# nintendops/DynamicFusion_Body

Hardware: AMD Instinct MI355X
Metric: Mvoxels/s TSDF fusion + GN-iters/s warp solve, 256³ grid, 1/2/4/8 GPU (higher is better)
Workload: dtype f64 geometry / f32 volume

## Files before the change

### dynamicfusion_body_amd/_lib.py

```python
import ctypes
import os
import re

_PKG = os.path.dirname(os.path.abspath(__file__))
LIB_PATH = os.environ.get("DFH_LIB_PATH") or os.path.join(_PKG, "libdfusion_hip.so")
HEADER_PATH = os.path.join(os.path.dirname(_PKG), "include", "dfusion_hip.h")

F32, F64 = 0, 1
ABI_VERSION = 8

_c_double_p = ctypes.POINTER(ctypes.c_double)
_c_int_p = ctypes.POINTER(ctypes.c_int)
_vp = ctypes.c_void_p
_int = ctypes.c_int
_dbl = ctypes.c_double


class Problem(ctypes.Structure):
    _fields_ = [("sample_pos", _vp), ("sample_nrm", _vp), ("nbr", _vp), ("weights", _vp), ("corr", _vp), ("valid", _vp),
                ("n_samples", _int), ("knn", _int),
                ("node_dq", _vp), ("node_pos", _vp), ("node_w", _vp), ("node_nbr", _vp), ("n_nodes", _int),
                ("lw_dq", _dbl * 8), ("rw", _dbl), ("huber_delta", _dbl),
                ("row_ptr", _vp), ("col", _vp), ("n_blocks", _int), ("vals", _vp), ("rhs", _vp), ("cost_count", _vp),
                ("blk_upper", _vp), ("n_upper", _int),
# ... 70 lines not shown
    "dfh_integrate_depth": (_int, [_volume_p, ctypes.POINTER(DepthViews), _dbl, _dbl, _c_double_p, _vp, ctypes.c_size_t, _vp]),
    "dfh_integrate_depth_path": (_int, [_int, _slab_p, _int, _int, _int]),
    "dfh_integrate_depth_ocl": (_int, [_volume_p, _vp, _int, _int, ctypes.POINTER(ctypes.c_float), ctypes.POINTER(ctypes.c_float), ctypes.c_float, ctypes.c_float, _vp]),
    "dfh_fuse_volume_rigid": (_int, [_volume_p, ctypes.POINTER(Live), _c_double_p, _dbl, _dbl, _vp]),
    "dfh_dqb_workspace_bytes": (ctypes.c_size_t, [_slab_p]),
    "dfh_dqb_workspace_bytes_cached": (ctypes.c_size_t, [_slab_p, _int, _int, _int]),
    "dfh_fuse_volume_dqb": (_int, [_volume_p, ctypes.POINTER(Live), ctypes.POINTER(Nodes), _c_double_p, _dbl, _dbl, _vp, ctypes.c_size_t, _int, _vp]),
    "dfh_integrate_depth_dqb": (_int, [_volume_p, ctypes.POINTER(DepthViews), ctypes.POINTER(Nodes), _c_double_p, _dbl, _dbl, _int, _vp,
                                      ctypes.c_size_t, _int, _vp]),
    "dfh_residual_rigid": (_int, [_vp, _vp, _vp, _int, _c_double_p, _vp, _vp]),
    "dfh_gn_build_rigid": (_int, [_vp, _vp, _vp, _vp, _int, _c_double_p, _vp, _vp]),
    "dfh_residual_data": (_int, [_vp, _vp, _vp, _vp, _int, _int, _vp, _vp, _vp, _int, _c_double_p, _vp, _vp]),
    "dfh_residual_reg": (_int, [_vp, _int, _int, _vp, _vp, _vp, _dbl, _vp, _vp]),
    "dfh_warp_points": (_int, [_vp, _vp, _vp, _int, _int, _vp, _vp, _vp, _int, _c_double_p, _vp, _vp, _vp]),
    "dfh_closest_correspondences": (_int, [_vp, _vp, _int, _vp, _int, _int, _dbl, _vp, _vp, _vp, _vp]),
    "dfh_nearest_points": (_int, [_vp, _int, _vp, _int, _vp, _vp, _vp]),
    "dfh_graph_unsupported": (_int, [_vp, _int, _vp, _int, _vp, _vp, _int, _vp, _vp]),
    "dfh_dq_blend_points": (_int, [_vp, _int, _vp, _int, _vp, _vp, _vp, _int, _vp, _vp]),
    "dfh_radius_sample_workspace_bytes": (ctypes.c_size_t, [ctypes.c_long]),
    "dfh_radius_sample": (_int, [_vp, ctypes.c_long, _dbl, _vp, ctypes.c_long, ctypes.POINTER(ctypes.c_long), _c_int_p, _vp,
                                 ctypes.c_size_t, _vp]),
    "dfh_sample_knn": (_int, [_vp, _int, _vp, _vp, _int, _int, _vp, _vp, _vp]),
    "dfh_dqb_skip_layout": (_int, [_slab_p, _c_int_p, _int, _int, ctypes.POINTER(ctypes.c_size_t)]),
    "dfh_dqb_build_candidates": (_int, [_slab_p, _vp, _int, _int, _vp, ctypes.c_size_t, _vp]),
    "dfh_sample_knn_bricks": (_int, [_vp, _int, _vp, _vp, _int, _int, _slab_p, _vp, ctypes.c_size_t, _vp, _vp, _vp]),
    "dfh_permute_samples": (_int, [_vp, _int, _int, _vp, _vp, _vp, _vp, _vp, _vp, _vp, _vp, _vp]),
    "dfh_gn_partial_doubles": (ctypes.c_size_t, [_int]),
    "dfh_gn_views_bytes": (ctypes.c_size_t, [_int, _int, _int, _int]),
    "dfh_gn_pack_views": (_int, [_vp, _int, ctypes.POINTER(ctypes.c_void_p), _int, _int, _int, _c_double_p, _vp]),
    "dfh_gn_associate": (_int, [_problem_p, _frame_p, _vp]),
    "dfh_gn_associate_volume": (_int, [_problem_p, _term_p, _vp]),
    "dfh_gn_build": (_int, [_problem_p, _frame_p, _vp]),
    "dfh_gn_build_volume": (_int, [_problem_p, _term_p, _vp]),
    "dfh_gn_solve": (_int, [_problem_p, _frame_p, ctypes.POINTER(SolveParams), _vp]),
    "dfh_gn_solve_volume": (_int, [_problem_p, _term_p, ctypes.POINTER(SolveParams), _vp]),
    "dfh_gn_associate_gated": (_int, [_problem_p, _frame_p, _gate_p, _vp]),
    "dfh_gn_build_gated": (_int, [_problem_p, _frame_p, _gate_p, _vp]),
    "dfh_gn_solve_gated": (_int, [_problem_p, _frame_p, _gate_p, ctypes.POINTER(SolveParams), _vp]),
    "dfh_gn_global_sampled_gated": (_int, [_problem_p, _frame_p, _gate_p, _int, _dbl, _int, _vp, _vp, _vp, ctypes.c_size_t, _vp]),
    "dfh_gn_pack_upper": (_int, [_vp, _vp, _vp, _vp, _int, _int, _int, _vp, _vp]),
    "dfh_gn_unpack_upper": (_int, [_vp, _vp, _vp, _vp, _int, _int, _int, _vp, _vp]),
    "dfh_gn_sort_workspace_bytes": (ctypes.c_size_t, [_int]),
    "dfh_gn_sort_samples": (_int, [_vp, _vp, _vp, _vp, _int, _int, _int, _vp, _vp, _vp, _vp, _vp, _vp, _vp, ctypes.c_size_t, _vp]),
    "dfh_gn_tile_samples": (_int, []),
    "dfh_gn_plan_count": (_int, [_vp, _int, _int, _vp, _vp, _vp]),
    "dfh_gn_plan_workspace_bytes": (ctypes.c_size_t, [_int, _int]),
# ... 134 lines not shown
```

### dynamicfusion_body_amd/csrc/dfh_fuse_volume.hip

```cpp
#include "dfh_dqb_front.h"

#include <algorithm>
#include <cmath>
#include <cstdlib>
#include <mutex>
#include <unordered_map>

namespace dfh {

template <typename T, int N>
struct alignas(sizeof(T) * N) VPack {
    T v[N];
};

struct RigidParams {
    DQ lw;
    double tdist, wmax;
    int X, Y, Z;
    int LX, LY, LZ;
    int x0, nx;
    int zpacks, zp_shift;
};

__device__ __forceinline__ void pack_coords2(int zpacks, int zp_shift, int &y, int &zp) {
// ... 701 lines not shown
        if (DFH_K3_STUB & 16) in.idx = make_uint2((unsigned)(r & 255) | 0x10000u * ((r + 7) & 255), (unsigned)((r + 3) & 255) | 0x10000u * ((r + 11) & 255));
        else in.idx = *reinterpret_cast<const uint2 *>(knn_cache + off * 4);
        if (DFH_K3_STUB & 4) { in.w0 = 0.4 + 1e-9 * lane; in.w1 = 0.3; in.w2 = 0.2; in.wi = 30.0f; }
        else {
            in.w0 = w_cache[off]; in.w1 = w_cache[nvox + off]; in.w2 = w_cache[2 * nvox + off];
            in.wi = wi_cache[off];
        }
        in.t = tsdf[off]; in.w = tsdf_w[off];
    };
    auto coords = [&](int r, double &px, double &py, double &pz) {
        const int row = r / runs_per_row;
        const int xl = row / p.Y;
        px = (double)(p.x0 + xl); py = (double)(row - xl * p.Y); pz = (double)((r - row * runs_per_row) * 64 + lane);
    };
    auto nodes_of = [&](uint2 idx, int (&bi)[4]) {
        bi[0] = min((int)(idx.x & 0xffffu), p.N - 1); bi[1] = min((int)(idx.x >> 16), p.N - 1);
        bi[2] = min((int)(idx.y & 0xffffu), p.N - 1); bi[3] = min((int)(idx.y >> 16), p.N - 1);
    };
    if (LIST) {
        const int l = wave % kSkipLists, first = wave / kSkipLists, step = max(n_waves / kSkipLists, 1);
        if (wave >= step * kSkipLists) return;
        const unsigned *__restrict__ mine = list + (size_t)l * sub_cap;
        const int n_entries = (int)min(list_count[16 * l], sub_cap);
        const int n_items = 16 * ((n_entries + 3) >> 2);
        const unsigned last_brick = (unsigned)(p.nbx * p.nby * p.nbz - 1);
        const int g = lane >> 4;
        auto entry_of = [&](int it) { const int e = 4 * (it >> 4) + g; return e < n_entries ? min(mine[e], last_brick) : 0xffffffffu; };
        unsigned entry = first < n_items ? entry_of(first) : 0xffffffffu;
        for (int it = first; it < n_items; it += step) {
            const unsigned brick = entry;
            if (it + step < n_items) entry = entry_of(it + step);
            const int rr = it & 15;
            const bool have = brick != 0xffffffffu;
            const unsigned bq = have ? brick : 0u;
            const int bz = (int)(bq % (unsigned)p.nbz), bxy = (int)(bq / (unsigned)p.nbz);
            const int by = bxy % p.nby, bx = bxy / p.nby;
            const int xl = bx * kBX + (rr >> 2), y = by * kBY + (rr & 3);
            const bool valid = have && xl < p.nx && y < p.Y;
            const size_t off = ((size_t)xl * p.Y + y) * p.Z + (size_t)(bz * kBZ + (lane & 15));
            const double px = (double)(p.x0 + xl), py = (double)y, pz = (double)(bz * kBZ + (lane & 15));
            DqbRunInputs in;
            in.idx = make_uint2(0u, 0u); in.w0 = 1.0; in.w1 = in.w2 = 0.0; in.wi = 1.0f; in.t = in.w = 0.0f;
            if (valid) {
                in.idx = *reinterpret_cast<const uint2 *>(knn_cache + off * 4);
                in.w0 = w_cache[off]; in.w1 = w_cache[nvox + off]; in.w2 = w_cache[2 * nvox + off];
                in.wi = wi_cache[off];
                in.t = tsdf[off]; in.w = tsdf_w[off];
            }
            int bi[4];
            nodes_of(in.idx, bi);
            DqbNorm e;
            e.w0 = in.w0; e.w1 = in.w1; e.w2 = in.w2; e.wi = in.wi;
            DqbWarped wp = dqb_stage_warp(DqLds<STRIDE>{sdq}, bi, e, p, f, px, py, pz);
            if (!valid) { wp.ok = false; wp.redo = false; wp.fx = wp.fy = wp.fz = 0.0; }
            LiveT c[8];
            dqb_stage_gather(live, p, wp, c);
            dqb_stage_finish<LiveT, true>(tsdf, tsdf_w, live, node_pos, node_dq, node_w, bi, e.wi, p, wp, c, px, py, pz, off, in.t, in.w, redo_list);
        }
        return;
    }
    if (wave >= n_runs) return;
    for (int r = wave; r < n_runs; r += n_waves) {
        DqbRunInputs in;
// ... 23 lines not shown
        const size_t off = redo_list.offs[i];
        const int z = (int)(off % (size_t)p.Z);
        const int y = (int)((off / (size_t)p.Z) % (size_t)p.Y);
        const int xl = (int)(off / ((size_t)p.Z * p.Y));
        const uint2 v = *reinterpret_cast<const uint2 *>(knn_cache + off * 4);
        int bi[4];
        bi[0] = min((int)(v.x & 0xffffu), p.N - 1); bi[1] = min((int)(v.x >> 16), p.N - 1);
        bi[2] = min((int)(v.y & 0xffffu), p.N - 1); bi[3] = min((int)(v.y >> 16), p.N - 1);
        dqb_exact_voxel(tsdf, tsdf_w, live, node_pos, node_dq, node_w, bi, p, (double)(p.x0 + xl), (double)y, (double)z, off, wi_cache[off]);
    }
    __syncthreads();
    if (threadIdx.x == 0 && atomicAdd(redo_list.count + 1, 1u) == gridDim.x - 1) {
        redo_list.count[0] = 0u;
        redo_list.count[1] = 0u;
    }
}

struct DqbSkip {
    unsigned long long *U;
    unsigned long long *S;
    unsigned char *mb;
    float *db;
    unsigned short *used;
    unsigned *sub_count;
    unsigned *sub_list;
    unsigned sub_cap;
    int CX, CY, CZ, WZ;
    int SCX, SCY;
};
constexpr int kSkipMaxWords = 8;
constexpr int kSkipUsed = 16;

template <typename LiveT>
__global__ __launch_bounds__(1024) void dqb_live_mask_kernel(const LiveT *__restrict__ live, int LX, int LY, int LZ, double tdist,
                                                              const DqbSkip k, int cx_lo) {
    __shared__ unsigned long long part[16][kSkipMaxWords];
    const int cell_row = cx_lo * k.CY + blockIdx.x;
    const int cx = cell_row / k.CY, cy = cell_row - cx * k.CY;
    const int wave = threadIdx.x >> 6, lane = threadIdx.x & 63;
    const int x = 4 * cx + (wave >> 2), y = 4 * cy + (wave & 3);
    const bool row_ok = x < LX && y < LY;
    for (int wz = 0; wz < k.WZ; ++wz) {
        const int cz = wz * 64 + lane;
        bool f = false;
        if (row_ok && cz < k.CZ) {
            const VPack<LiveT, 4> v = *reinterpret_cast<const VPack<LiveT, 4> *>(live + ((size_t)x * LY + y) * LZ + 4 * (size_t)cz);
// ... 57 lines not shown
    int base = 0;
    for (int w = 0; w < wave; ++w) base += wave_cnt[w];
    const int total = wave_cnt[0] + wave_cnt[1] + wave_cnt[2] + wave_cnt[3];
    if (total > kSkipUsed) {
        if (threadIdx.x < kSkipUsed) out[threadIdx.x] = threadIdx.x == 0 ? (unsigned short)0xfffe : (unsigned short)0xffff;
        return;
    }
    if ((int)threadIdx.x >= total && threadIdx.x < kSkipUsed) out[threadIdx.x] = (unsigned short)0xffff;
    if (f) out[base + __builtin_popcountll(m & ((1ull << lane) - 1ull))] = (unsigned short)slist[threadIdx.x];
}

__device__ __forceinline__ unsigned long long row_shr(unsigned long long cur, unsigned long long nxt, int s) { return (cur >> s) | (nxt << (64 - s)); }
__device__ __forceinline__ unsigned long long row_shl(unsigned long long cur, unsigned long long prv, int s) { return (cur << s) | (prv >> (64 - s)); }
__device__ __forceinline__ unsigned long long wave_and_u64(unsigned long long v) {
    unsigned lo = (unsigned)v, hi = (unsigned)(v >> 32);
#pragma unroll
    for (int o = 32; o >= 1; o >>= 1) {
        lo &= (unsigned)__shfl_xor((int)lo, o, 64);
        hi &= (unsigned)__shfl_xor((int)hi, o, 64);
    }
    return ((unsigned long long)hi << 32) | lo;
}

__global__ __launch_bounds__(256) void dqb_reach_kernel(const DqbParams p, const DqbSkip k) {
    const int t = blockIdx.x * 4 + (threadIdx.x >> 6);
    if (t >= k.SCX * k.SCY) return;
    const int lane = threadIdx.x & 63;
    const int scx = t / k.SCY, cy = t - scx * k.SCY;
    const int cx = p.x0 / 4 + scx;
    const int dx = lane / 5 - 2, dy = lane % 5 - 2;
    const bool nb = lane < 25;
    const int ax = cx + dx, ay = cy + dy;
    const bool inside = nb && ax >= 0 && ax < k.CX && ay >= 0 && ay < k.CY;
    const unsigned long long *urow = k.U + ((size_t)(inside ? ax : 0) * k.CY + (inside ? ay : 0)) * k.WZ;
    unsigned char *rs = k.mb + ((long)scx * p.nby + cy) * p.nbz;
    for (int wz = 0; wz < k.WZ; ++wz) {
        unsigned long long e1 = ~0ull, e2 = ~0ull;
        if (nb) {
            const unsigned long long cur = inside ? urow[wz] : 0ull, prv = inside && wz > 0 ? urow[wz - 1] : 0ull,
                                     nxt = inside && wz + 1 < k.WZ ? urow[wz + 1] : 0ull;
            const unsigned long long a1 = cur & row_shr(cur, nxt, 1) & row_shl(cur, prv, 1);
            e2 = a1 & row_shr(cur, nxt, 2) & row_shl(cur, prv, 2);
            if (dx >= -1 && dx <= 1 && dy >= -1 && dy <= 1) e1 = a1;
        }
        e1 = wave_and_u64(e1);
        e2 = wave_and_u64(e2);
        if (lane < 16) {
            const int bz = wz * 16 + lane;
            const unsigned long long grp = 0xfull << (4 * lane);
            if (bz < p.nbz) rs[bz] = (e2 & grp) == grp ? 2 : ((e1 & grp) == grp ? 1 : 0);
        }
    }
    for (int bz = k.WZ * 16 + lane; bz < p.nbz; bz += 64) rs[bz] = 0;
}

__global__ __launch_bounds__(256) void dqb_bound_kernel(const double *__restrict__ node_dq, const DqbParams p, const DqbSkip k, int all_bounds) {
    __shared__ float sq[16][kSkipUsed * 15 + 1];
    const long nbricks = (long)p.nbx * p.nby * p.nbz;
    const long brick_raw = (long)blockIdx.x * 16 + (threadIdx.x >> 4);
    const bool real = brick_raw < nbricks;
    const long brick = real ? brick_raw : 0;
    const int grp = threadIdx.x >> 4, sub = threadIdx.x & 15;
    const int bz = (int)(brick % p.nbz);
    const int by = (int)((brick / p.nbz) % p.nby);
    const int bx = (int)(brick / ((long)p.nbz * p.nby));
    const double cxd = (double)(p.x0 + bx * kBX) + 0.5 * (kBX - 1), cyd = (double)(by * kBY) + 0.5 * (kBY - 1),
                 czd = (double)(bz * kBZ) + 0.5 * (kBZ - 1);
    const float cx = (float)cxd, cy = (float)cyd, cz = (float)czd;
    const int rs = real ? (int)k.mb[brick] : 0;
    const bool want = real && (rs > 0 || all_bounds);
    const unsigned short id = want ? k.used[brick * kSkipUsed + sub] : (unsigned short)0xffff;
    const bool have = id < 0xfffe && (int)id < p.N;
    bool bad = false;
    float me[8] = {1.0f, 0.0f, 0.0f, 0.0f, 0.0f, 0.0f, 0.0f, 0.0f};
    if (have) {
#pragma unroll
        for (int c8 = 0; c8 < 8; ++c8) me[c8] = (float)node_dq[8 * (size_t)id + c8];
    }
    float *mine = &sq[grp][sub * 15];
#pragma unroll
    for (int c8 = 0; c8 < 8; ++c8) {
        mine[c8] = me[c8];
        bad = bad | !(fabsf(me[c8]) < 1e6f);
    }
    mine[8] = -(me[1] * cx + me[2] * cy + me[3] * cz);
    mine[9] = me[0] * cx + me[2] * cz - me[3] * cy;
    mine[10] = me[0] * cy + me[3] * cx - me[1] * cz;
    mine[11] = me[0] * cz + me[1] * cy - me[2] * cx;
    const float vv = (me[1] * me[1] + me[2] * me[2]) + me[3] * me[3];
    mine[12] = sqrtf(vv);
    mine[13] = sqrtf((me[0] - 1.0f) * (me[0] - 1.0f) + vv);
    const int n = __builtin_popcount((unsigned)(__ballot(have) >> (16 * (grp & 3))) & 0xffffu);
    const bool overflow = (__shfl((int)id, (int)(threadIdx.x & 48), 64) & 0xffff) == 0xfffe;
// ... 16 lines not shown
        const float t2x = -b0 * ax + b1 * aw - b2 * az + b3 * ay, t2y = -b0 * ay + b2 * aw - b3 * ax + b1 * az, t2z = -b0 * az + b3 * aw - b1 * ay + b2 * ax;
        const float rr = (aw * bw + ax * bx_) + (ay * by_ + az * bz_), dd = (a0 * b0 + a1 * b1) + (a2 * b2 + a3 * b3);
        const float gx = 0.5f * (s1x + s2x) - (rr + dd) * cx + (t1x + t2x);
        const float gy = 0.5f * (s1y + s2y) - (rr + dd) * cy + (t1y + t2y);
        const float gz = 0.5f * (s1z + s2z) - (rr + dd) * cz + (t1z + t2z);
        const float lam = a[12] + b[12] + 2.0f * a[13] * b[13] + fabsf(dd);
        num = fmaxf(num, sqrtf(gx * gx + gy * gy + gz * gz) + lam * (float)DFH_BRICK_RADIUS);
        n2min = fminf(n2min, rr);
    }
#pragma unroll
    for (int o = 8; o >= 1; o >>= 1) {
        num = fmaxf(num, __shfl_xor(num, o, 16));
        n2min = fminf(n2min, __shfl_xor(n2min, o, 16));
        bad = bad | (__shfl_xor(bad ? 1 : 0, o, 16) != 0);
    }
    float D = __builtin_huge_valf();
    int m = 255;
    if (want && !overflow && n >= 1 && !bad && n2min > 0.25f && num < 1e6f) {
        const double cn = sqrt((cxd * cxd + cyd * cyd) + czd * czd) + DFH_BRICK_RADIUS;
        double d = (double)num / ((double)n2min * (1.0 - 1e-5)) * (1.0 + 1e-5);
        d = d + (cn + d) * 0x1p-23 + cn * 4e-6 + 2e-3;
        D = (float)(d * (1.0 + 0x1p-22));
        const double need = d + 1.0;
        m = need <= 4.0 ? 1 : (need <= 8.0 ? 2 : 255);
    }
    const bool safe = m <= rs && all_bounds != 2;
    if (sub == 0 && real) {
        k.db[brick] = want ? D : -1.0f;
        k.mb[brick] = (unsigned char)m;
        reinterpret_cast<unsigned char *>(k.S)[brick] = safe ? 1 : 0;
    }
    const unsigned l = (blockIdx.x ^ (blockIdx.x >> 6) ^ (blockIdx.x >> 12) ^ (blockIdx.x >> 18)) % kSkipLists;
    const unsigned long long unsafe = __ballot(sub == 0 && real && !safe);
    if (unsafe == 0ull) return;
    const int lane = threadIdx.x & 63;
    unsigned base = 0;
    if (lane == __builtin_ctzll(unsafe)) base = atomicAdd(k.sub_count + 16 * l, (unsigned)__builtin_popcountll(unsafe));
    base = (unsigned)__builtin_amdgcn_readlane((int)base, __builtin_ctzll(unsafe));
    if (sub == 0 && real && !safe)
        k.sub_list[(size_t)l * k.sub_cap + base + (unsigned)__builtin_popcountll(unsafe & ((1ull << lane) - 1ull))] = (unsigned)brick;
}

template <bool NT>
__global__ __launch_bounds__(256) void dqb_stream_kernel(float *__restrict__ tsdf, float *__restrict__ tsdf_w, const float *__restrict__ wi_cache,
                                                          const DqbParams p, const DqbSkip k, const DqbRedoList redo_list, unsigned npacks, int sat_ok) {
    const unsigned pack = blockIdx.x * 256u + threadIdx.x;
    if (pack >= npacks) return;
    const unsigned zp = (unsigned)p.Z >> 2;
    const unsigned row = pack / zp, cz = pack - row * zp;
    const unsigned xl = row / (unsigned)p.Y, y = row - xl * (unsigned)p.Y;
    if (!reinterpret_cast<const unsigned char *>(k.S)[((size_t)(xl >> 2) * p.nby + (y >> 2)) * p.nbz + (cz >> 2)]) return;
    const size_t off = (size_t)pack * 4;
    typedef float v4f __attribute__((ext_vector_type(4)));
    float4 t0, w0;
    if (NT) {
        const v4f a = __builtin_nontemporal_load(reinterpret_cast<const v4f *>(tsdf + off)), b = __builtin_nontemporal_load(reinterpret_cast<const v4f *>(tsdf_w + off));
        t0 = make_float4(a.x, a.y, a.z, a.w); w0 = make_float4(b.x, b.y, b.z, b.w);
    } else {
        t0 = *reinterpret_cast<const float4 *>(tsdf + off);
        w0 = *reinterpret_cast<const float4 *>(tsdf_w + off);
    }
    const float td = (float)p.tdist, wm = (float)p.wmax;
    if (sat_ok && t0.x == td && t0.y == td && t0.z == td && t0.w == td && w0.x == wm && w0.y == wm && w0.z == wm && w0.w == wm) return;
    float4 wi;
    if (NT) { const v4f c = __builtin_nontemporal_load(reinterpret_cast<const v4f *>(wi_cache + off)); wi = make_float4(c.x, c.y, c.z, c.w); }
    else wi = *reinterpret_cast<const float4 *>(wi_cache + off);
    float4 t = t0, w = w0;
    float *tv = &t.x, *wv = &w.x;
    const float *wiv = &wi.x;
#pragma unroll
    for (int j = 0; j < 4; ++j) {
        if (wiv[j] >= 0.0f) {
            dqb_update_f32(tv[j], wv[j], wiv[j], p.tdist, p.wmax, tv[j], wv[j]);
        } else {
// ... 2 lines not shown
    }
    if (t.x != t0.x || t.y != t0.y || t.z != t0.z || t.w != t0.w) {
        if (NT) { v4f a; a.x = t.x; a.y = t.y; a.z = t.z; a.w = t.w; __builtin_nontemporal_store(a, reinterpret_cast<v4f *>(tsdf + off)); }
        else *reinterpret_cast<float4 *>(tsdf + off) = t;
    }
    if (w.x != w0.x || w.y != w0.y || w.z != w0.z || w.w != w0.w) {
        if (NT) { v4f a; a.x = w.x; a.y = w.y; a.z = w.z; a.w = w.w; __builtin_nontemporal_store(a, reinterpret_cast<v4f *>(tsdf_w + off)); }
        else *reinterpret_cast<float4 *>(tsdf_w + off) = w;
    }
}

static bool skip_layout(const DqbParams &p, double *w_cache, DqbSkip &k, size_t *used = nullptr) {
    const size_t nv = (size_t)p.nx * p.Y * p.Z;
    k.CX = (p.LX + 3) / 4; k.CY = (p.LY + 3) / 4; k.CZ = p.LZ / 4; k.WZ = (k.CZ + 63) / 64;
    k.SCX = p.nx / 4; k.SCY = (p.Y + 3) / 4;
    const long nbricks = (long)p.nbx * p.nby * p.nbz;
    char *base = reinterpret_cast<char *>(w_cache);
    size_t at = (nv * 32 + 16 + 63) & ~(size_t)63;
    auto take = [&](size_t bytes) { char *q = base ? base + at : nullptr; at = (at + bytes + 63) & ~(size_t)63; return q; };
    k.used = reinterpret_cast<unsigned short *>(take((size_t)nbricks * kSkipUsed * 2));
    k.U = reinterpret_cast<unsigned long long *>(take((size_t)k.CX * k.CY * k.WZ * 8));
    k.S = reinterpret_cast<unsigned long long *>(take((size_t)nbricks));
    k.mb = reinterpret_cast<unsigned char *>(take((size_t)nbricks));
    k.sub_cap = (unsigned)((((nbricks + 15) / 16 + kSkipLists - 1) / kSkipLists) * 16);
    k.sub_count = reinterpret_cast<unsigned *>(take((size_t)kSkipLists * 64));
    k.sub_list = reinterpret_cast<unsigned *>(take((size_t)kSkipLists * k.sub_cap * 4));
    k.db = reinterpret_cast<float *>(take((size_t)nbricks * 4));
    if (used) *used = at;
    return at <= nv * 40;
}

static bool skip_sizes_ok(const DqbParams &p) {
    const size_t nv = (size_t)p.nx * p.Y * p.Z;
    return p.x0 % 4 == 0 && p.nx % 4 == 0 && p.LZ % 4 == 0 && p.LZ <= 64 * 4 * kSkipMaxWords && p.Z % 64 == 0 && p.Z <= 2048 &&
           nv / 4 < (1ull << 32);
}

template <typename LiveT>
static int launch_dqb_fast(void *tsdf, void *tsdf_w, const void *live, const double *node_pos, const double *node_dq,
                           const double *node_w, int *cand, unsigned short *knn_cache, double *w_cache, int mode, const DqbParams &p,
                           hipStream_t s) {
    RigidFastParams f;
    fold_rigid(p.lw.q, f);
    DqbRedoList redo_list{nullptr, nullptr};
    if (w_cache) {
        const size_t nv = (size_t)p.nx * p.Y * p.Z;
        unsigned *base = reinterpret_cast<unsigned *>(reinterpret_cast<char *>(w_cache) + nv * 28);
        redo_list.count = base;
        redo_list.offs = base + 4;
        if (mode == 1) DFH_HIP_CHECK(hipMemsetAsync(base, 0, 16, s));
// ... 25 lines not shown
        DeviceInfo &di = device_info(dev);
        if (di.n_cu == 0) DFH_HIP_CHECK(hipDeviceGetAttribute(&di.n_cu, hipDeviceAttributeMultiprocessorCount, dev));
        const int tpb = (opt().k3_tpb == 256 || opt().k3_tpb == 512) && !big ? (int)opt().k3_tpb : 1024;
        long per_cu = (long)(160 * 1024 / (lds + 512));
        const long max_per_cu = 2048 / tpb;
        if (per_cu > max_per_cu) per_cu = max_per_cu;
        if (opt().k3_wg_per_cu > 0 && opt().k3_wg_per_cu < per_cu) per_cu = opt().k3_wg_per_cu;
        long wgs = per_cu * di.n_cu;
        const int wpb = tpb / 64;
        if (wgs * wpb > n_runs) wgs = (n_runs + wpb - 1) / wpb;
        DqbSkip sk = {};
        const size_t nv = (size_t)p.nx * p.Y * p.Z;
        const bool skip_wanted = opt().k3_skip > 0 || (opt().k3_skip < 0 && (long)p.X * p.Y * p.Z > (1L << 24));
        bool skip = skip_wanted && p.tdist > 0.0 && (double)(float)p.tdist == p.tdist && skip_sizes_ok(p) &&
                    (uintptr_t)live % (4 * sizeof(LiveT)) == 0 && (uintptr_t)tsdf % 16 == 0 && (uintptr_t)tsdf_w % 16 == 0 &&
                    p.lw.q[0] == 1.0 && p.lw.q[1] == 0.0 && p.lw.q[2] == 0.0 && p.lw.q[3] == 0.0 && p.lw.q[4] == 0.0 && p.lw.q[5] == 0.0 &&
                    p.lw.q[6] == 0.0 && p.lw.q[7] == 0.0;
        if (skip) skip = skip_layout(p, w_cache, sk);
        const float *wi_cache = reinterpret_cast<const float *>(w_cache + 3 * nv);
        if (skip) {
            const long nbr = (long)p.nbx * p.nby * p.nbz;
            int ex = 0;
            const int sat_ok = frexp(p.tdist, &ex) == 0.5 && p.wmax > 0.0 && (double)(float)p.wmax == p.wmax ? 1 : 0;
            const int cx_lo = std::max(0, p.x0 / 4 - 2), cx_hi = std::min(sk.CX, (p.x0 + p.nx) / 4 + 2);
            if (cx_hi > cx_lo)
                hipLaunchKernelGGL((dqb_live_mask_kernel<LiveT>), dim3((unsigned)((cx_hi - cx_lo) * sk.CY)), dim3(1024), 0, s, (const LiveT *)live, p.LX,
                                   p.LY, p.LZ, p.tdist, sk, cx_lo);
            hipLaunchKernelGGL(dqb_reach_kernel, dim3((unsigned)((sk.SCX * sk.SCY + 3) / 4)), dim3(256), 0, s, p, sk);
            hipLaunchKernelGGL(dqb_bound_kernel, dim3((unsigned)((nbr + 15) / 16)), dim3(256), 0, s, node_dq, p, sk, opt().k3_skip == 2 ? 1 : (opt().k3_skip == 3 ? 2 : 0));
            if (nv * 8 > ((size_t)256 << 20))
                hipLaunchKernelGGL(dqb_stream_kernel<true>, dim3((unsigned)((nv / 4 + 255) / 256)), dim3(256), 0, s, (float *)tsdf, (float *)tsdf_w, wi_cache,
                                   p, sk, redo_list, (unsigned)(nv / 4), sat_ok);
            else
                hipLaunchKernelGGL(dqb_stream_kernel<false>, dim3((unsigned)((nv / 4 + 255) / 256)), dim3(256), 0, s, (float *)tsdf, (float *)tsdf_w, wi_cache,
                                   p, sk, redo_list, (unsigned)(nv / 4), sat_ok);
        }
#define DFH_K3L(TPB, STRIDE)                                                                                                                          \
        do {                                                                                                                                          \
            if (skip) hipLaunchKernelGGL((fuse_volume_dqb_lds_kernel<LiveT, TPB, STRIDE, true>), dim3((unsigned)wgs), dim3(TPB), lds, s, (float *)tsdf,  \
                                         (float *)tsdf_w, (const LiveT *)live, node_pos, node_dq, node_w, knn_cache, w_cache, p, f, (int)n_runs,        \
                                         redo_list, (const unsigned *)sk.sub_count, (const unsigned *)sk.sub_list, sk.sub_cap);                       \
            else hipLaunchKernelGGL((fuse_volume_dqb_lds_kernel<LiveT, TPB, STRIDE, false>), dim3((unsigned)wgs), dim3(TPB), lds, s, (float *)tsdf,     \
                                    (float *)tsdf_w, (const LiveT *)live, node_pos, node_dq, node_w, knn_cache, w_cache, p, f, (int)n_runs, redo_list, \
                                    (const unsigned *)nullptr, (const unsigned *)nullptr, 0u);                                                       \
        } while (0)
        if (big) DFH_K3L(1024, kDqLdsStrideBig);
        else if (tpb == 256) DFH_K3L(256, kDqLdsStride); else if (tpb == 512) DFH_K3L(512, kDqLdsStride); else DFH_K3L(1024, kDqLdsStride);
// ... 231 lines not shown
extern "C" int dfh_dqb_skip_layout(const dfh_slab *slab, const int live_res[3], int knn, int n_nodes, size_t out[13]) {
    using namespace dfh;
    const int rc = check_slab("dfh_dqb_skip_layout", slab);
    if (rc != DFH_OK) return rc;
    DFH_REQUIRE(live_res && out, "dfh_dqb_skip_layout: null pointer");
    DFH_REQUIRE(knn == 4, "dfh_dqb_skip_layout: the skip belongs to the knn = 4 float32 path");
    for (int i = 0; i < 13; ++i) out[i] = 0;
    if (slab->x1 == slab->x0) return DFH_OK;
    const DqbParams p = dqb_params(*slab, live_res, n_nodes, knn);
    const size_t cached1 = dfh_dqb_workspace_bytes_cached(slab, knn, n_nodes, 1);
    const size_t cached2 = dfh_dqb_workspace_bytes_cached(slab, knn, n_nodes, 2);
    DFH_REQUIRE(cached2 > cached1, "dfh_dqb_skip_layout: no level-2 workspace for these sizes");
    DqbSkip k = {};
    size_t used = 0;
    const bool fits = skip_layout(p, reinterpret_cast<double *>(cached1), k, &used);
    out[0] = reinterpret_cast<size_t>(k.U); out[1] = reinterpret_cast<size_t>(k.S); out[2] = reinterpret_cast<size_t>(k.mb);
    out[3] = reinterpret_cast<size_t>(k.db);
    out[6] = (size_t)k.CX; out[7] = (size_t)k.CY; out[8] = (size_t)k.WZ; out[9] = (size_t)k.SCX; out[10] = (size_t)k.SCY;
    out[11] = fits && skip_sizes_ok(p) ? 1 : 0;
    out[12] = reinterpret_cast<size_t>(k.used);
    return DFH_OK;
}

extern "C" int dfh_dqb_build_candidates(const dfh_slab *slab, const double *node_pos, int n_nodes, int knn,
                                        void *workspace, size_t workspace_bytes, void *stream) {
    using namespace dfh;
    const int rc = check_slab("dfh_dqb_build_candidates", slab);
    if (rc != DFH_OK) return rc;
    DFH_REQUIRE(node_pos, "dfh_dqb_build_candidates: null pointer");
    DFH_REQUIRE(knn >= 1 && knn <= kKMax && n_nodes >= knn, "dfh_dqb_build_candidates: knn=%d, %d nodes", knn, n_nodes);
    if (slab->x1 == slab->x0) return DFH_OK;
    DFH_REQUIRE(workspace && workspace_bytes >= dfh_dqb_workspace_bytes(slab),
                "dfh_dqb_build_candidates: workspace too small (need %zu bytes)", dfh_dqb_workspace_bytes(slab));
    const DqbParams p = dqb_params(*slab, nullptr, n_nodes, knn);
    const long nbricks = (long)p.nbx * p.nby * p.nbz;
    DFH_REQUIRE(nbricks < (1L << 31), "dfh_dqb_build_candidates: too many bricks");
    hipLaunchKernelGGL(dqb_candidates_kernel, dim3((unsigned)((nbricks + 255) / 256)), dim3(256), 0, static_cast<hipStream_t>(stream),
                       node_pos, static_cast<int *>(workspace), p);
    DFH_HIP_CHECK(hipGetLastError());
    return DFH_OK;
}

extern "C" int dfh_sample_knn_bricks(const double *sample_pos, int n_samples, const double *node_pos, const double *node_w,
                                     int n_nodes, int knn, const dfh_slab *slab, const void *workspace,
                                     size_t workspace_bytes, int *nbr_out, double *weights_out, void *stream) {
    using namespace dfh;
// ... 22 lines not shown
```

### dynamicfusion_body_amd/kernels.py

```python
import ctypes
import numpy as np
import torch

from . import _lib
from .device import current_stream_ptr, dtype_code, require_gpu


def _check_volume_pair(T, Wt, res, x_range):
    if not (isinstance(T, torch.Tensor) and isinstance(Wt, torch.Tensor)):
        raise ValueError("volumes must be torch tensors on the GPU")
    if not (T.is_cuda and Wt.is_cuda):
        raise ValueError("volumes must live on the GPU")
    if T.dtype != Wt.dtype:
        raise ValueError("tsdf and weight volumes must share a dtype")
    if not (T.is_contiguous() and Wt.is_contiguous()):
        raise ValueError("volumes must be contiguous [x][y][z]")
    x0, x1 = x_range
    want = (x1 - x0, res[1], res[2])
    if tuple(T.shape) != want or tuple(Wt.shape) != want:
        raise ValueError("volume shape %s / %s does not match slab %s of grid %s"
                         % (tuple(T.shape), tuple(Wt.shape), want, tuple(res)))


def _volume(T, Wt, res, x_range, tsdf_res=None):
# ... 159 lines not shown
    else:
        nbytes = lib.dfh_dqb_workspace_bytes(_lib.slab(res, x_range))
    return torch.empty(max(1, (nbytes + 3) // 4), dtype=torch.int32, device=device or "cuda")


def dqb_skip_tables(workspace, res, live_res, n_nodes, x_range=None, knn=4):
    lib = _lib.load()
    if x_range is None:
        x_range = (0, res[0])
    out = (ctypes.c_size_t * 13)()
    _lib.check(lib.dfh_dqb_skip_layout(_lib.slab(res, x_range), _lib.iarr(live_res), int(knn), int(n_nodes), out), "dfh_dqb_skip_layout")
    raw = workspace.view(torch.uint8)
    nx = int(x_range[1]) - int(x_range[0])
    nb = (-(-nx // 4)) * (-(-int(res[1]) // 4)) * (-(-int(res[2]) // 16))
    CX, CY, WZ, SCX, SCY = (int(out[i]) for i in (6, 7, 8, 9, 10))
    n_runs = nx * int(res[1]) * (int(res[2]) // 16)

    def region(i, nbytes, dtype):
        return raw[int(out[i]):int(out[i]) + nbytes].view(dtype)
    tabs = {"ok": bool(out[11]), "U": region(0, CX * CY * WZ * 8, torch.int64).view(CX, CY, WZ), "S": region(1, nb, torch.uint8),
            "reach": region(2, nb, torch.uint8), "bound": region(3, nb * 4, torch.float32), "used": region(12, nb * 32, torch.int16).view(nb, 16)}
    tabs["n_runs"] = n_runs
    tabs["n_listed"] = int((tabs["S"] == 0).sum()) * 16
    return tabs


def dqb_build_candidates(workspace, res, node_pos, knn, x_range=None):
    require_gpu()
    lib = _lib.load()
    P = node_pos if isinstance(node_pos, torch.Tensor) else torch.from_numpy(np.ascontiguousarray(np.asarray(node_pos, dtype=np.float64)))
    P = P.to(device="cuda", dtype=torch.float64).contiguous()
    _lib.check(lib.dfh_dqb_build_candidates(_lib.slab(res, x_range), P.data_ptr(), int(P.shape[0]), int(knn), workspace.data_ptr(),
                                            workspace.numel() * 4, current_stream_ptr()), "dfh_dqb_build_candidates")
    return workspace


def _node_tensors(node_pos, node_dq, node_w):
    def prep(a, shape_tail):
        t = a if isinstance(a, torch.Tensor) else torch.from_numpy(np.ascontiguousarray(np.asarray(a, dtype=np.float64)))
        t = t.to(device="cuda", dtype=torch.float64).contiguous()
        if tuple(t.shape[1:]) != shape_tail:
            raise ValueError("node array has shape %s, expected (N,%s)" % (tuple(t.shape), ",".join(map(str, shape_tail))))
        return t
    P, Q, Wn = prep(node_pos, (3,)), prep(node_dq, (8,)), prep(node_w, ())
    if not (P.shape[0] == Q.shape[0] == Wn.shape[0]):
        raise ValueError("node_pos / node_dq / node_w disagree on the number of nodes")
# ... 135 lines not shown
```

### include/dfusion_hip.h

```cpp
#ifndef DFUSION_HIP_H
#define DFUSION_HIP_H

#include <stddef.h>
#include <stdint.h>

#ifdef __cplusplus
extern "C" {
#endif

#define DFH_ABI_VERSION 8

#define DFH_F32 0
#define DFH_F64 1

#define DFH_OK 0
#define DFH_E_BADARG (-1)
#define DFH_E_HIP (-2)
#define DFH_E_UNSUPPORTED (-3)
#define DFH_E_TIMEOUT (-4)
#define DFH_E_INTERNAL (-5)

int dfh_version(void);

const char *dfh_last_error(void);
// ... 48 lines not shown
                       double *out, void *stream);

int dfh_gn_build_rigid(const double *verts, const double *normals, const double *corr, const unsigned char *valid, int n,
                       const double x[8], double *out44, void *stream);

int dfh_residual_data(const double *verts, const double *normals, const double *corr, const int *nbr, int n_verts,
                      int knn, const double *node_dq, const double *node_pos, const double *node_w, int n_nodes,
                      const double lw_dq[8], double *out, void *stream);

int dfh_residual_reg(const int *node_nbr, int n_nodes, int knn, const double *node_dq, const double *node_pos,
                     const double *node_w, double rw, double *out, void *stream);

int dfh_warp_points(const double *verts, const double *normals, const int *nbr, int n_verts, int knn, const double *node_dq,
                    const double *node_pos, const double *node_w, int n_nodes, const double lw_dq[8], double *out_pos,
                    double *out_nrm, void *stream);

int dfh_closest_correspondences(const double *warped_pos, const double *warped_nrm, int n_verts, const double *live_verts,
                                int n_live, int knn, double tolerance, double *corr_out, double *cost_out,
                                unsigned char *keep_out, void *stream);

int dfh_sample_knn(const double *sample_pos, int n_samples, const double *node_pos, const double *node_w, int n_nodes,
                   int knn, int *nbr_out, double *weights_out, void *stream);
int dfh_dqb_skip_layout(const dfh_slab *slab, const int live_res[3], int knn, int n_nodes, size_t out[13]);
int dfh_dqb_build_candidates(const dfh_slab *slab, const double *node_pos, int n_nodes, int knn,
                             void *workspace, size_t workspace_bytes, void *stream);
int dfh_sample_knn_bricks(const double *sample_pos, int n_samples, const double *node_pos, const double *node_w,
                          int n_nodes, int knn, const dfh_slab *slab, const void *workspace,
                          size_t workspace_bytes, int *nbr_out, double *weights_out, void *stream);

int dfh_nearest_points(const double *query, int n_query, const double *cloud, int n_cloud, int *idx_out, double *d2_out, void *stream);
int dfh_graph_unsupported(const double *verts, int n_verts, const int *nbr, int knn, const double *node_pos, const double *node_w,
                          int n_nodes, unsigned char *flag_out, void *stream);
int dfh_dq_blend_points(const double *points, int n_points, const int *nbr, int knn, const double *node_dq, const double *node_pos,
                        const double *node_w, int n_nodes, double *dq_out, void *stream);

size_t dfh_radius_sample_workspace_bytes(long n_points);
int dfh_radius_sample(const double *points, long n_points, double radius, int *idx_out, long capacity, long *count_out,
                      int *rounds_out, void *workspace, size_t workspace_bytes, void *stream);

int dfh_permute_samples(const long *order, int n_samples, int knn, const double *pos, const double *nrm, const int *nbr,
                        const double *weights, double *pos_out, double *nrm_out, int *nbr_out, double *weights_out, void *stream);

typedef struct dfh_gn_problem {
    const double *sample_pos, *sample_nrm;
    const int *nbr;
    const double *weights;
// ... 180 lines not shown
```

Baseline: 500,700.

## Refine DQB skip to per-z-cell granularity with larger reach

Splits the per-brick safe-skip decision into four z-cells per brick, each with its own reach level (now up to 3 bricks instead of 2). Only unsafe cells are put on the work lists, and the list-processing loop handles 4-voxel z-cells instead of 16-voxel brick rows. The aim is to skip more voxels whose deformation bound allows the cheap path, so fewer voxels go through the full dual-quaternion blend. In exchange the reach kernel does more wave reductions, the lists grow fourfold, and the list loop gives each 4-lane group its own cell, which hurts coalescing.

```diff
diff --git a/dynamicfusion_body_amd/_lib.py b/dynamicfusion_body_amd/_lib.py
--- a/dynamicfusion_body_amd/_lib.py
+++ b/dynamicfusion_body_amd/_lib.py
@@ -116,6 +116,7 @@
                                  ctypes.c_size_t, _vp]),
     "dfh_sample_knn": (_int, [_vp, _int, _vp, _vp, _int, _int, _vp, _vp, _vp]),
     "dfh_dqb_skip_layout": (_int, [_slab_p, _c_int_p, _int, _int, ctypes.POINTER(ctypes.c_size_t)]),
+    "dfh_dqb_skip_layout_cells": (_int, [_slab_p, _c_int_p, _int, _int, ctypes.POINTER(ctypes.c_size_t)]),
     "dfh_dqb_build_candidates": (_int, [_slab_p, _vp, _int, _int, _vp, ctypes.c_size_t, _vp]),
     "dfh_sample_knn_bricks": (_int, [_vp, _int, _vp, _vp, _int, _int, _slab_p, _vp, ctypes.c_size_t, _vp, _vp, _vp]),
     "dfh_permute_samples": (_int, [_vp, _int, _int, _vp, _vp, _vp, _vp, _vp, _vp, _vp, _vp, _vp]),
diff --git a/dynamicfusion_body_amd/csrc/dfh_fuse_volume.hip b/dynamicfusion_body_amd/csrc/dfh_fuse_volume.hip
--- a/dynamicfusion_body_amd/csrc/dfh_fuse_volume.hip
+++ b/dynamicfusion_body_amd/csrc/dfh_fuse_volume.hip
@@ -747,23 +747,24 @@
         if (wave >= step * kSkipLists) return;
         const unsigned *__restrict__ mine = list + (size_t)l * sub_cap;
         const int n_entries = (int)min(list_count[16 * l], sub_cap);
-        const int n_items = 16 * ((n_entries + 3) >> 2);
-        const unsigned last_brick = (unsigned)(p.nbx * p.nby * p.nbz - 1);
-        const int g = lane >> 4;
-        auto entry_of = [&](int it) { const int e = 4 * (it >> 4) + g; return e < n_entries ? min(mine[e], last_brick) : 0xffffffffu; };
+        const int n_items = 16 * ((n_entries + 15) >> 4);
+        const unsigned last_cell = 4u * (unsigned)(p.nbx * p.nby * p.nbz) - 1u;
+        const int g = lane >> 2;
+        auto entry_of = [&](int it) { const int e = 16 * (it >> 4) + g; return e < n_entries ? min(mine[e], last_cell) : 0xffffffffu; };
         unsigned entry = first < n_items ? entry_of(first) : 0xffffffffu;
         for (int it = first; it < n_items; it += step) {
-            const unsigned brick = entry;
+            const unsigned cell = entry;
             if (it + step < n_items) entry = entry_of(it + step);
             const int rr = it & 15;
-            const bool have = brick != 0xffffffffu;
-            const unsigned bq = have ? brick : 0u;
+            const bool have = cell != 0xffffffffu;
+            const unsigned bq = have ? cell >> 2 : 0u;
+            const int zc = (int)(have ? cell & 3u : 0u) * 4 + (lane & 3);
             const int bz = (int)(bq % (unsigned)p.nbz), bxy = (int)(bq / (unsigned)p.nbz);
             const int by = bxy % p.nby, bx = bxy / p.nby;
             const int xl = bx * kBX + (rr >> 2), y = by * kBY + (rr & 3);
             const bool valid = have && xl < p.nx && y < p.Y;
-            const size_t off = ((size_t)xl * p.Y + y) * p.Z + (size_t)(bz * kBZ + (lane & 15));
-            const double px = (double)(p.x0 + xl), py = (double)y, pz = (double)(bz * kBZ + (lane & 15));
+            const size_t off = ((size_t)xl * p.Y + y) * p.Z + (size_t)(bz * kBZ + zc);
+            const double px = (double)(p.x0 + xl), py = (double)y, pz = (double)(bz * kBZ + zc);
             DqbRunInputs in;
             in.idx = make_uint2(0u, 0u); in.w0 = 1.0; in.w1 = in.w2 = 0.0; in.wi = 1.0f; in.t = in.w = 0.0f;
             if (valid) {
@@ -833,6 +834,8 @@
     unsigned char *mb;
     float *db;
     unsigned short *used;
+    unsigned char *cs;
+    unsigned char *rc;
     unsigned *sub_count;
     unsigned *sub_list;
     unsigned sub_cap;
@@ -936,36 +939,48 @@
     return ((unsigned long long)hi << 32) | lo;
 }
 
+constexpr int kSkipReach = 3;
 __global__ __launch_bounds__(256) void dqb_reach_kernel(const DqbParams p, const DqbSkip k) {
     const int t = blockIdx.x * 4 + (threadIdx.x >> 6);
     if (t >= k.SCX * k.SCY) return;
     const int lane = threadIdx.x & 63;
     const int scx = t / k.SCY, cy = t - scx * k.SCY;
     const int cx = p.x0 / 4 + scx;
-    const int dx = lane / 5 - 2, dy = lane % 5 - 2;
-    const bool nb = lane < 25;
+    constexpr int W = 2 * kSkipReach + 1;
+    const int dx = lane / W - kSkipReach, dy = lane % W - kSkipReach;
+    const bool nb = lane < W * W;
+    const int ring = max(abs(dx), abs(dy));
     const int ax = cx + dx, ay = cy + dy;
     const bool inside = nb && ax >= 0 && ax < k.CX && ay >= 0 && ay < k.CY;
     const unsigned long long *urow = k.U + ((size_t)(inside ? ax : 0) * k.CY + (inside ? ay : 0)) * k.WZ;
-    unsigned char *rs = k.mb + ((long)scx * p.nby + cy) * p.nbz;
+    unsigned char *rcell = k.rc + ((long)scx * p.nby + cy) * p.nbz;
     for (int wz = 0; wz < k.WZ; ++wz) {
-        unsigned long long e1 = ~0ull, e2 = ~0ull;
+        unsigned long long e1 = ~0ull, e2 = ~0ull, e3 = ~0ull;
         if (nb) {
             const unsigned long long cur = inside ? urow[wz] : 0ull, prv = inside && wz > 0 ? urow[wz - 1] : 0ull,
                                      nxt = inside && wz + 1 < k.WZ ? urow[wz + 1] : 0ull;
             const unsigned long long a1 = cur & row_shr(cur, nxt, 1) & row_shl(cur, prv, 1);
-            e2 = a1 & row_shr(cur, nxt, 2) & row_shl(cur, prv, 2);
-            if (dx >= -1 && dx <= 1 && dy >= -1 && dy <= 1) e1 = a1;
+            const unsigned long long a2 = a1 & row_shr(cur, nxt, 2) & row_shl(cur, prv, 2);
+            e3 = a2 & row_shr(cur, nxt, 3) & row_shl(cur, prv, 3);
+            if (ring <= 2) e2 = a2;
+            if (ring <= 1) e1 = a1;
         }
         e1 = wave_and_u64(e1);
         e2 = wave_and_u64(e2);
+        e3 = wave_and_u64(e3);
         if (lane < 16) {
             const int bz = wz * 16 + lane;
-            const unsigned long long grp = 0xfull << (4 * lane);
-            if (bz < p.nbz) rs[bz] = (e2 & grp) == grp ? 2 : ((e1 & grp) == grp ? 1 : 0);
-        }
-    }
-    for (int bz = k.WZ * 16 + lane; bz < p.nbz; bz += 64) rs[bz] = 0;
+            const unsigned g1 = (unsigned)(e1 >> (4 * lane)) & 0xfu, g2 = (unsigned)(e2 >> (4 * lane)) & 0xfu,
+                           g3 = (unsigned)(e3 >> (4 * lane)) & 0xfu;
+            if (bz < p.nbz) {
+                unsigned r = 0;
+#pragma unroll
+                for (int c = 0; c < 4; ++c) r |= (((g1 >> c) & 1u) + ((g2 >> c) & 1u) + ((g3 >> c) & 1u)) << (2 * c);
+                rcell[bz] = (unsigned char)r;
+            }
+        }
+    }
+    for (int bz = k.WZ * 16 + lane; bz < p.nbz; bz += 64) rcell[bz] = 0;
 }
 
 __global__ __launch_bounds__(256) void dqb_bound_kernel(const double *__restrict__ node_dq, const DqbParams p, const DqbSkip k, int all_bounds) {
@@ -981,8 +996,8 @@
     const double cxd = (double)(p.x0 + bx * kBX) + 0.5 * (kBX - 1), cyd = (double)(by * kBY) + 0.5 * (kBY - 1),
                  czd = (double)(bz * kBZ) + 0.5 * (kBZ - 1);
     const float cx = (float)cxd, cy = (float)cyd, cz = (float)czd;
-    const int rs = real ? (int)k.mb[brick] : 0;
-    const bool want = real && (rs > 0 || all_bounds);
+    const unsigned rcb = real ? (unsigned)k.rc[brick] : 0u;
+    const bool want = real && (rcb != 0u || all_bounds);
     const unsigned short id = want ? k.used[brick * kSkipUsed + sub] : (unsigned short)0xffff;
     const bool have = id < 0xfffe && (int)id < p.N;
     bool bad = false;
@@ -1045,23 +1060,37 @@
         d = d + (cn + d) * 0x1p-23 + cn * 4e-6 + 2e-3;
         D = (float)(d * (1.0 + 0x1p-22));
         const double need = d + 1.0;
-        m = need <= 4.0 ? 1 : (need <= 8.0 ? 2 : 255);
-    }
-    const bool safe = m <= rs && all_bounds != 2;
+        m = need <= 4.0 ? 1 : (need <= 8.0 ? 2 : (need <= 4.0 * kSkipReach ? 3 : 255));
+    }
+    unsigned safe_cells = 0u;
+    if (all_bounds != 2) {
+#pragma unroll
+        for (int c = 0; c < 4; ++c) safe_cells |= (m <= (int)((rcb >> (2 * c)) & 3u) ? 1u : 0u) << c;
+    }
     if (sub == 0 && real) {
         k.db[brick] = want ? D : -1.0f;
         k.mb[brick] = (unsigned char)m;
-        reinterpret_cast<unsigned char *>(k.S)[brick] = safe ? 1 : 0;
+        reinterpret_cast<unsigned char *>(k.S)[brick] = safe_cells == 0xfu ? 1 : 0;
+        k.cs[brick] = (unsigned char)safe_cells;
     }
     const unsigned l = (blockIdx.x ^ (blockIdx.x >> 6) ^ (blockIdx.x >> 12) ^ (blockIdx.x >> 18)) % kSkipLists;
-    const unsigned long long unsafe = __ballot(sub == 0 && real && !safe);
-    if (unsafe == 0ull) return;
+    const unsigned unsafe_cells = sub == 0 && real ? ~safe_cells & 0xfu : 0u;
+    const int n_mine = __builtin_popcount(unsafe_cells);
+    const int n0 = __builtin_amdgcn_readlane(n_mine, 0), n1 = __builtin_amdgcn_readlane(n_mine, 16), n2 = __builtin_amdgcn_readlane(n_mine, 32),
+              n3 = __builtin_amdgcn_readlane(n_mine, 48);
+    const int total = n0 + n1 + n2 + n3;
+    if (total == 0) return;
     const int lane = threadIdx.x & 63;
     unsigned base = 0;
-    if (lane == __builtin_ctzll(unsafe)) base = atomicAdd(k.sub_count + 16 * l, (unsigned)__builtin_popcountll(unsafe));
-    base = (unsigned)__builtin_amdgcn_readlane((int)base, __builtin_ctzll(unsafe));
-    if (sub == 0 && real && !safe)
-        k.sub_list[(size_t)l * k.sub_cap + base + (unsigned)__builtin_popcountll(unsafe & ((1ull << lane) - 1ull))] = (unsigned)brick;
+    if (lane == 0) base = atomicAdd(k.sub_count + 16 * l, (unsigned)total);
+    base = (unsigned)__builtin_amdgcn_readlane((int)base, 0);
+    if (unsafe_cells) {
+        const int g4 = grp & 3;
+        unsigned at = base + (unsigned)((g4 > 0 ? n0 : 0) + (g4 > 1 ? n1 : 0) + (g4 > 2 ? n2 : 0));
+#pragma unroll
+        for (int c = 0; c < 4; ++c)
+            if ((unsafe_cells >> c) & 1u) k.sub_list[(size_t)l * k.sub_cap + at++] = 4u * (unsigned)brick + (unsigned)c;
+    }
 }
 
 template <bool NT>
@@ -1072,7 +1101,7 @@
     const unsigned zp = (unsigned)p.Z >> 2;
     const unsigned row = pack / zp, cz = pack - row * zp;
     const unsigned xl = row / (unsigned)p.Y, y = row - xl * (unsigned)p.Y;
-    if (!reinterpret_cast<const unsigned char *>(k.S)[((size_t)(xl >> 2) * p.nby + (y >> 2)) * p.nbz + (cz >> 2)]) return;
+    if (!((k.cs[((size_t)(xl >> 2) * p.nby + (y >> 2)) * p.nbz + (cz >> 2)] >> (cz & 3u)) & 1u)) return;
     const size_t off = (size_t)pack * 4;
     typedef float v4f __attribute__((ext_vector_type(4)));
     float4 t0, w0;
@@ -1121,10 +1150,12 @@
     k.U = reinterpret_cast<unsigned long long *>(take((size_t)k.CX * k.CY * k.WZ * 8));
     k.S = reinterpret_cast<unsigned long long *>(take((size_t)nbricks));
     k.mb = reinterpret_cast<unsigned char *>(take((size_t)nbricks));
-    k.sub_cap = (unsigned)((((nbricks + 15) / 16 + kSkipLists - 1) / kSkipLists) * 16);
+    k.sub_cap = (unsigned)((((nbricks + 15) / 16 + kSkipLists - 1) / kSkipLists) * 16 * 4);
     k.sub_count = reinterpret_cast<unsigned *>(take((size_t)kSkipLists * 64));
     k.sub_list = reinterpret_cast<unsigned *>(take((size_t)kSkipLists * k.sub_cap * 4));
     k.db = reinterpret_cast<float *>(take((size_t)nbricks * 4));
+    k.cs = reinterpret_cast<unsigned char *>(take((size_t)nbricks));
+    k.rc = reinterpret_cast<unsigned char *>(take((size_t)nbricks));
     if (used) *used = at;
     return at <= nv * 40;
 }
@@ -1196,7 +1227,7 @@
             const long nbr = (long)p.nbx * p.nby * p.nbz;
             int ex = 0;
             const int sat_ok = frexp(p.tdist, &ex) == 0.5 && p.wmax > 0.0 && (double)(float)p.wmax == p.wmax ? 1 : 0;
-            const int cx_lo = std::max(0, p.x0 / 4 - 2), cx_hi = std::min(sk.CX, (p.x0 + p.nx) / 4 + 2);
+            const int cx_lo = std::max(0, p.x0 / 4 - kSkipReach), cx_hi = std::min(sk.CX, (p.x0 + p.nx) / 4 + kSkipReach);
             if (cx_hi > cx_lo)
                 hipLaunchKernelGGL((dqb_live_mask_kernel<LiveT>), dim3((unsigned)((cx_hi - cx_lo) * sk.CY)), dim3(1024), 0, s, (const LiveT *)live, p.LX,
                                    p.LY, p.LZ, p.tdist, sk, cx_lo);
@@ -1474,6 +1505,26 @@
     return DFH_OK;
 }
 
+extern "C" int dfh_dqb_skip_layout_cells(const dfh_slab *slab, const int live_res[3], int knn, int n_nodes, size_t out[5]) {
+    using namespace dfh;
+    const int rc = check_slab("dfh_dqb_skip_layout_cells", slab);
+    if (rc != DFH_OK) return rc;
+    DFH_REQUIRE(live_res && out, "dfh_dqb_skip_layout_cells: null pointer");
+    DFH_REQUIRE(knn == 4, "dfh_dqb_skip_layout_cells: the skip belongs to the knn = 4 float32 path");
+    for (int i = 0; i < 5; ++i) out[i] = 0;
+    if (slab->x1 == slab->x0) return DFH_OK;
+    const DqbParams p = dqb_params(*slab, live_res, n_nodes, knn);
+    const size_t cached1 = dfh_dqb_workspace_bytes_cached(slab, knn, n_nodes, 1);
+    const size_t cached2 = dfh_dqb_workspace_bytes_cached(slab, knn, n_nodes, 2);
+    DFH_REQUIRE(cached2 > cached1, "dfh_dqb_skip_layout_cells: no level-2 workspace for these sizes");
+    DqbSkip k = {};
+    skip_layout(p, reinterpret_cast<double *>(cached1), k);
+    out[0] = reinterpret_cast<size_t>(k.cs); out[1] = reinterpret_cast<size_t>(k.rc);
+    out[2] = reinterpret_cast<size_t>(k.sub_count); out[3] = reinterpret_cast<size_t>(k.sub_list);
+    out[4] = (size_t)k.sub_cap;
+    return DFH_OK;
+}
+
 extern "C" int dfh_dqb_build_candidates(const dfh_slab *slab, const double *node_pos, int n_nodes, int knn,
                                         void *workspace, size_t workspace_bytes, void *stream) {
     using namespace dfh;
diff --git a/dynamicfusion_body_amd/kernels.py b/dynamicfusion_body_amd/kernels.py
--- a/dynamicfusion_body_amd/kernels.py
+++ b/dynamicfusion_body_amd/kernels.py
@@ -205,6 +205,14 @@
             "reach": region(2, nb, torch.uint8), "bound": region(3, nb * 4, torch.float32), "used": region(12, nb * 32, torch.int16).view(nb, 16)}
     tabs["n_runs"] = n_runs
     tabs["n_listed"] = int((tabs["S"] == 0).sum()) * 16
+    oc = (ctypes.c_size_t * 5)()
+    _lib.check(lib.dfh_dqb_skip_layout_cells(_lib.slab(res, x_range), _lib.iarr(live_res), int(knn), int(n_nodes), oc),
+               "dfh_dqb_skip_layout_cells")
+    cap = int(oc[4])
+    tabs["cells"] = raw[int(oc[0]):int(oc[0]) + nb]
+    tabs["cell_reach"] = raw[int(oc[1]):int(oc[1]) + nb]
+    tabs["sub_count"] = raw[int(oc[2]):int(oc[2]) + 64 * 64].view(torch.int32).view(64, 16)[:, 0]
+    tabs["sub_list"] = raw[int(oc[3]):int(oc[3]) + 64 * cap * 4].view(torch.int32).view(64, cap)
     return tabs
 
 
diff --git a/include/dfusion_hip.h b/include/dfusion_hip.h
--- a/include/dfusion_hip.h
+++ b/include/dfusion_hip.h
@@ -94,6 +94,7 @@
 int dfh_sample_knn(const double *sample_pos, int n_samples, const double *node_pos, const double *node_w, int n_nodes,
                    int knn, int *nbr_out, double *weights_out, void *stream);
 int dfh_dqb_skip_layout(const dfh_slab *slab, const int live_res[3], int knn, int n_nodes, size_t out[13]);
+int dfh_dqb_skip_layout_cells(const dfh_slab *slab, const int live_res[3], int knn, int n_nodes, size_t out[5]);
 int dfh_dqb_build_candidates(const dfh_slab *slab, const double *node_pos, int n_nodes, int knn,
                              void *workspace, size_t workspace_bytes, void *stream);
 int dfh_sample_knn_bricks(const double *sample_pos, int n_samples, const double *node_pos, const double *node_w,
```

New measurement: 501,100, median of 2. About the same (+0.1%).
